# sumansamui/CMOOP_Audio_Processing

Measured on AMD Instinct MI355X. Metric: candidate-net evals/hour (pop=40, GSC-v2), higher is better.
Workload: dtype f32

## Files before the change

cmoop_audio_processing_amd/_lib.py:

```python
from __future__ import annotations

import ctypes as C
import os
import re
import subprocess
import threading

_HERE = os.path.dirname(os.path.abspath(__file__))
CSRC = os.path.join(_HERE, "csrc")
LIB_PATH = os.environ.get("CMOOP_LIB_PATH") or os.path.join(CSRC, "libcmoop_hip.so")
HEADER = os.path.join(os.path.dirname(_HERE), "include", "cmoop.h")

_lock = threading.Lock()
_lib = None


class CmoopError(RuntimeError):
    pass


class Config(C.Structure):
    _fields_ = [(n, C.c_int32) for n in (
        "variant", "classes", "epochs", "batch", "patience", "early_stop", "restore_best", "acc_readout",
        "fpr_variant", "shuffle", "eval_batch", "n_slots", "profile_every", "gemm_mode")] + \
        [(n, C.c_double) for n in ("lr", "beta1", "beta2", "adam_eps", "bn_eps", "bn_momentum", "dropout")]


class DatasetStruct(C.Structure):
    _fields_ = [("x_train", C.c_void_p), ("y_train", C.c_void_p), ("n_train", C.c_int64),
                ("x_val", C.c_void_p), ("y_val", C.c_void_p), ("n_val", C.c_int64),
                ("T", C.c_int32), ("F", C.c_int32)]


NEXT_FN = C.CFUNCTYPE(C.c_int32, C.c_void_p)


STREAM_PROTOTYPES = {
    "cmoop_net_predict": [C.c_void_p, C.c_void_p, C.c_int64, C.c_void_p],
    "cmoop_logmel_stream": [C.c_void_p, C.c_void_p, C.c_int64, C.c_void_p],
    "cmoop_logmel_stream_time": [C.c_void_p, C.c_void_p, C.c_int64, C.c_void_p, C.c_int32, C.c_void_p],
    "cmoop_stream_windows": [C.c_int64, C.c_int32, C.c_int32, C.c_void_p],
    "cmoop_net_predict_stream": [C.c_void_p, C.c_void_p, C.c_int64, C.c_int32, C.c_void_p, C.c_void_p, C.c_void_p, C.c_void_p],
}


def build(verbose: bool = False) -> str:
    jobs = str(min(8, os.cpu_count() or 1))
    r = subprocess.run(["make", "-C", CSRC, "-j", jobs], capture_output=True, text=True)
    if r.returncode != 0:
        raise CmoopError("building libcmoop_hip.so failed:\n" + r.stdout[-4000:] + r.stderr[-4000:])
    if verbose:
        print(r.stdout[-2000:])
    return LIB_PATH


def declared_symbols():
    txt = open(HEADER).read()
    return sorted(set(re.findall(r"\b(cmoop_[a-z0-9_]+)\s*\(", txt)))


def lib():
    global _lib
    with _lock:
        if _lib is not None:
            return _lib
        if not os.path.exists(LIB_PATH):
            raise CmoopError(
                f"{LIB_PATH} is missing: run `python -c 'import __graft_entry__ as g; g.build()'` "
                "(or `make -C cmoop_audio_processing_amd/csrc`). There is no CPU fallback for this path.")
        try:
            L = C.CDLL(LIB_PATH)
        except OSError as e:
            raise CmoopError(f"cannot load {LIB_PATH}: {e}") from e
        L.cmoop_last_error.restype = C.c_char_p
        L.cmoop_abi_version.restype = C.c_int
        for name in declared_symbols():
            fn = getattr(L, name)
            if name not in ("cmoop_last_error", "cmoop_config_default"):
                fn.restype = C.c_int
        L.cmoop_config_default.restype = None
        for name, argtypes in STREAM_PROTOTYPES.items():
            getattr(L, name).argtypes = argtypes
        _lib = L
        return L


def check(rc: int) -> None:
    if rc != 0:
        raise CmoopError(lib().cmoop_last_error().decode("utf-8", "replace"))


def default_config() -> Config:
    c = Config()
    lib().cmoop_config_default(C.byref(c))
    return c


def last_kernels():
    buf = C.create_string_buffer(1024)
    check(lib().cmoop_last_kernels(buf, C.c_int32(1024)))
    return [k for k in buf.value.decode().split(";") if k]


def profile_entries():
# ... 28 lines not shown
```

cmoop_audio_processing_amd/csrc/api.hip:

```cpp
#include "../../include/cmoop.h"
#include "net.h"

#include <cstring>
#include <memory>
#include <mutex>
#include <vector>

using namespace cmoop;

static thread_local std::string g_err;
static thread_local std::string g_last_kernels;

template <class F>
static int guard(F&& f) {
    try {
        f();
        return 0;
    } catch (const std::exception& e) {
        g_err = e.what();
        return 1;
    } catch (...) {
        g_err = "unknown error";
        return 2;
    }
// ... 739 lines not shown
                if (mfma_dgrad) {
                    CMOOP_HIP(hipMalloc(&wd, NK * 4));
                    launch_flip_transpose(w, wd, Cout, KS, KS, Cin, s);
                    if (KS * KS <= 32) {
                        tab_d_rows = rowtab_rows(gd);
                        CMOOP_HIP(hipMalloc(&tab_d, (size_t)tab_d_rows * 8));
                        launch_build_rowtab(gd, tab_d, s);
                    }
                    skf = igemm_splitk_workspace(gd);
                    if (skf) CMOOP_HIP(hipMalloc(&sk, skf * 4));
                }
                conv_backward_data(dy, w, dx, g, wd, mask_relu ? x : nullptr, 1.f, accumulate, s, &hook, sk, skf, GEMM_DEFAULT, mfma_dgrad,
                                   tab_d, tab_d_rows);
            }
            CMOOP_HIP(hipStreamSynchronize(s));
        } catch (...) {
            cleanup();
            throw;
        }
        cleanup();
    });
}

int cmoop_last_kernels(char* buf, int32_t cap) {
    return guard([&] {
        CMOOP_REQUIRE(buf && cap > 0, "last_kernels: no buffer");
        std::snprintf(buf, cap, "%s", g_last_kernels.c_str());
    });
}

int cmoop_conv_time(int32_t mode, const float* x, const float* w, const float* bias, float* y, int32_t B, int32_t H,
                    int32_t W, int32_t Cin, int32_t Cout, int32_t KS, int32_t iters, double* avg_ms) {
    return guard([&] {
        hipStream_t s = lib_stream();
        const ConvGeom g = make_geom(B, H, W, Cin, Cout, KS, 1);
        float *wd = nullptr, *wg = nullptr, *sk = nullptr;
        ConvGeom gd = g;
        GemmEpilogue e;
        const int S = wgrad_slices(g);
        if (mode == 0) e.bias = bias;
        if (mode == 1) {
            CMOOP_HIP(hipMalloc(&wd, (size_t)g.Cout * g.K() * 4));
            launch_flip_transpose(w, wd, Cout, KS, KS, Cin, s);
            gd.H = g.OH; gd.W = g.OW; gd.Cin = Cout; gd.Cout = Cin; gd.OH = g.H; gd.OW = g.W;
            gd.pad_t = KS - 1 - g.pad_t; gd.pad_l = KS - 1 - g.pad_l;
        }
// ... 68 lines not shown
```

cmoop_audio_processing_amd/csrc/gemm.hip:

```cpp
#include "kernels.h"
#include <hip/hip_ext.h>
#include <cstdlib>
#include <mutex>
#include <string>
#include <type_traits>

namespace cmoop {

typedef float f32x4 __attribute__((ext_vector_type(4)));

typedef __bf16 bf16x8 __attribute__((ext_vector_type(8)));
typedef unsigned u32x4 __attribute__((ext_vector_type(4)));

typedef __bf16 bf16x2 __attribute__((ext_vector_type(2)));
typedef float f32x2 __attribute__((ext_vector_type(2)));

template <int NP>
__device__ __forceinline__ void split_pair(const float x, const float y, unsigned (&w)[NP]) {
    if constexpr (NP == 1) {
        w[0] = __builtin_bit_cast(unsigned, __builtin_convertvector((f32x2){x, y}, bf16x2));
    } else {
        const unsigned ux = __float_as_uint(x), uy = __float_as_uint(y);
        w[0] = __builtin_amdgcn_perm(uy, ux, 0x07060302u);
        const float rx = x - __uint_as_float(ux & 0xFFFF0000u), ry = y - __uint_as_float(uy & 0xFFFF0000u);
// ... 1238 lines not shown
    if (c.halo) {
        c.mode = GEMM_FP32_HALO; c.use_dma = false;
        c.bm = halo_bm(cg.Cout);
        c.bn = std::min(cg.Cout, 64);
    } else if (halo_env && (c.mode == GEMM_FP32 || c.mode == GEMM_FP32_DMA) && c.bm == 128 && (c.splits > 1 || c.balanced_wgs) && ep.out_stride == 1) {
        int L = 0;
        const size_t need = halo_balanced_slab_floats(cg, &L);
        if (need > 0 && need <= ws_floats) {
            c.halo = true; c.halo_L = L; c.mode = GEMM_FP32_HALO; c.use_dma = false; c.stats = false;
            c.bm = 128; c.bn = 64; c.splits = 1; c.balanced_wgs = 512;
        }
    }
    c.flags = (c.splits > 1 ? GEMM_FLAG_SPLITK : 0) | (c.stats ? GEMM_FLAG_STATS : 0) | (c.balanced_wgs ? GEMM_FLAG_BALANCED : 0) |
              ((!c.halo && have_rowtab && (cg.Cin % bk) == 0 && cg.KH * cg.KW <= 32) ? GEMM_FLAG_ROWTAB : 0);
    return c;
}

int igemm_fwd_plan(const ConvGeom& g, const GemmEpilogue& ep, size_t ws_floats, bool want_stats, bool have_rowtab, int* flags_out) {
    igemm_check_range(g);
    CMOOP_REQUIRE(ilog2_exact(g.Cin) >= 4, "implicit GEMM needs C_in a power of two >= 16");
    const FwdChoice c = choose_fwd(g, ep, ws_floats, want_stats, have_rowtab);
    if (flags_out) *flags_out = c.flags;
    return c.code();
}

int launch_igemm_fwd(const float* X, const float* Wt, float* Y, const ConvGeom& cg, const GemmEpilogue& ep,
                     hipStream_t s, const GemmTiming* tm, float* splitk_ws, size_t splitk_ws_floats, int* stats_blocks,
                     const void* rowtab_v, int tab_rows, int* flags_out) {
    if (stats_blocks) *stats_blocks = 0;
    if (flags_out) *flags_out = 0;
    const uint2* rowtab = static_cast<const uint2*>(rowtab_v);
    GeomDev g = to_dev(cg);
    if (g.M == 0) return 0;
    EpiDev e;
    e.bias = ep.bias; e.mask = ep.mask; e.mask_scale = ep.mask_scale; e.relu = ep.relu;
    e.accumulate = ep.accumulate; e.out_stride = ep.out_stride; e.OHf = ep.OHf; e.OWf = ep.OWf;
    e.dropout = ep.dropout; e.drop_prefix = ep.drop_prefix; e.drop_thr = ep.drop_thr; e.drop_scale = ep.drop_scale;
    if (e.out_stride > 1)
        CMOOP_REQUIRE((int64_t)g.B * e.OHf * e.OWf * g.Cout < (1ll << 29), "scattered output too large");
    const FwdChoice ch = choose_fwd(cg, ep, splitk_ws ? splitk_ws_floats : 0, ep.stats != nullptr && stats_blocks != nullptr, rowtab != nullptr);
    const int mode = ch.mode == GEMM_FP32_DMA ? (int)GEMM_FP32 : ch.mode;
    const int bm = ch.bm, bn = ch.bn, splits = ch.splits, balanced_wgs = ch.balanced_wgs;
    const bool bk32_tile = ch.bk32_tile, use_dma = ch.use_dma;
    e.bal_L = 0; e.bal_segmax = 0;
    e.stats = ch.stats ? ep.stats : nullptr;
    if (e.stats) *stats_blocks = cdiv(g.M, bm);
// ... 902 lines not shown
```

cmoop_audio_processing_amd/csrc/kernels.h:

```cpp
#pragma once
#include "common.h"
#include <string>
#include <vector>

namespace cmoop {

struct ConvGeom {
    int B, H, W, Cin;
    int OH, OW, Cout;
    int KH, KW, stride;
    int pad_t, pad_l;
    int M() const { return B * OH * OW; }
    int K() const { return KH * KW * Cin; }
};

enum GemmMode { GEMM_DEFAULT = -1, GEMM_FP32 = 0, GEMM_FP32_DMA = 1 , GEMM_BF16X3 = 2, GEMM_BF16 = 3,
                GEMM_FP32_HALO = 4  };
int gemm_mode_default();

struct GemmEpilogue {
    int mode = GEMM_DEFAULT;
    const float* bias = nullptr;
    int relu = 0;
    const float* mask = nullptr;
    float mask_scale = 1.f;
    int accumulate = 0;
    int out_stride = 1;
    int OHf = 0, OWf = 0;
    int dropout = 0;
    uint32_t drop_prefix = 0, drop_thr = 0;
    float drop_scale = 1.f;
    float* stats = nullptr;
};

struct GemmTiming {
    hipEvent_t start = nullptr, stop = nullptr;
    bool ext = true;
};
enum GemmFlags { GEMM_FLAG_SPLITK = 1, GEMM_FLAG_STATS = 2, GEMM_FLAG_ROWTAB = 4, GEMM_FLAG_BALANCED = 8, GEMM_FLAG_SLABS = 16 };
int launch_igemm_fwd(const float* X, const float* Wt, float* Y, const ConvGeom& g,
                     const GemmEpilogue& e, hipStream_t s, const GemmTiming* tm = nullptr,
                     float* splitk_ws = nullptr, size_t splitk_ws_floats = 0, int* stats_blocks = nullptr,
                     const void* rowtab = nullptr, int tab_rows = 0, int* flags_out = nullptr);
size_t igemm_splitk_workspace(const ConvGeom& g);
int igemm_fwd_plan(const ConvGeom& g, const GemmEpilogue& e, size_t ws_floats, bool want_stats, bool have_rowtab, int* flags_out);
int igemm_wgrad_plan(const ConvGeom& g, int S, int mode, bool have_rowtab, int* flags_out);
void halo_rows_bound_and_need(const ConvGeom& g, int* bound, int* need, int* items_cap);
void igemm_check_range(const ConvGeom& g);
std::string gemm_kernel_name(int cls, int code);

int wgrad_slices(const ConvGeom& g);
int launch_igemm_wgrad(const float* X, const float* dY, float* P, const ConvGeom& g, int S, hipStream_t s,
                       const GemmTiming* tm = nullptr, float* Pbias = nullptr, size_t slab_stride = 0,
                       int mode = GEMM_DEFAULT, const void* rowtab = nullptr, int tab_rows = 0, int* flags_out = nullptr);
int rowtab_rows(const ConvGeom& g);
void launch_build_rowtab(const ConvGeom& g, void* tab, hipStream_t s);
void launch_reduce_slices(const float* P, float* out, int S, int64_t n, hipStream_t s, int64_t stride = 0);
void launch_flip_transpose(const float* W, float* Wd, int Cout, int KH, int KW, int Cin, hipStream_t s);
struct FlipEntry { int64_t w_off, wd_off; int Cout, KH, KW, Cin; };
void launch_flip_transpose_all(const float* params, float* wd_all, const FlipEntry* table_dev, int layers, int64_t max_elems,
                               hipStream_t s);

struct StepState {
    long long row0;
    unsigned step;
    unsigned iter;
};
void launch_step_advance(StepState* st, int batch, hipStream_t s);
void launch_glorot_init(float* w, int64_t n, uint32_t prefix, float scale, hipStream_t s);
void launch_fill(float* w, float v, int64_t n, hipStream_t s);

void launch_dense_fwd(const float* X, const float* W, const float* bias, float* Y, int M, int N, int K, int relu,
                      int dropout, uint32_t drop_prefix, uint32_t drop_thr, float drop_scale, int mode, hipStream_t s,
                      const StepState* st = nullptr, uint32_t drop_seed = 0, uint32_t drop_stream = 0);
void launch_dense_dgrad(const float* dY, const float* W, float* dX, int M, int N, int K, const float* mask, float mask_scale,
                        int mode, hipStream_t s);
void launch_dense_wgrad(const float* X, const float* dY, float* dW, float* dB, int M, int N, int K, int mode, hipStream_t s);
void launch_dense_bwd(const float* X, const float* dY, const float* W, float* dW, float* dB, float* dX, int M, int N, int K,
                      const float* mask, float mask_scale, int mode, hipStream_t s);

void launch_conv1_fwd(const float* X, const int32_t* idx, int64_t row0, const float* Wt, const float* bias,
                      float* Y, int B, int H, int W, int Cout, int KS, int relu, hipStream_t s, const StepState* st = nullptr,
                      int64_t n_rows = 0, float* stats = nullptr, int* stats_blocks = nullptr);
int conv1_wgrad_blocks(int B, int H, int W);
void launch_conv1_wgrad(const float* X, const int32_t* idx, int64_t row0, const float* dY, float* P,
                        int B, int H, int W, int Cout, int KS, hipStream_t s, const StepState* st = nullptr, int64_t n_rows = 0);

int colreduce_blocks(int64_t M, int C);
void launch_colstats(const float* X, float* P, int64_t M, int C, int blocks, hipStream_t s);
void launch_bn_bwd_reduce(const float* dY, const float* X, const float* mean, const float* invstd,
                          float* P, int64_t M, int C, int blocks, hipStream_t s);
void launch_bn_finalize(const float* P, int blocks, int64_t M, int C, const float* gamma, const float* beta,
                        float* moving_mean, float* moving_var, float* mean, float* invstd, float* scale,
// ... 82 lines not shown
```

cmoop_audio_processing_amd/csrc/net.h:

```cpp
#pragma once
#include "kernels.h"
#include <atomic>
#include <functional>
#include <map>
#include <mutex>
#include <set>
#include <string>
#include <vector>

namespace cmoop {

struct NetConfig {
    int variant = 0, classes = 10, epochs = 300, batch = 64, patience = 5;
    int early_stop = 1, restore_best = 0, acc_readout = 0, fpr_variant = 0, shuffle = 1;
    int eval_batch = 256, n_slots = 8, profile_every = 0;
    int gemm_mode = GEMM_FP32;
    double lr = 1e-3, beta1 = 0.9, beta2 = 0.999, adam_eps = 1e-7, bn_eps = 1e-3, bn_momentum = 0.99, dropout = 0.3;
};

struct Dataset {
    const float* x_train = nullptr; const int32_t* y_train = nullptr; int64_t n_train = 0;
    const float* x_val = nullptr;   const int32_t* y_val = nullptr;   int64_t n_val = 0;
    int T = 0, F = 0;
};
// ... 45 lines not shown
struct Op {
    OpKind kind;
    int in = -1, in2 = -1, out = -1;
    int KS = 1, stride = 1, Cin = 0, Cout = 0;
    int relu = 0, need_dgrad = 1, in_is_relu = 0, dgrad_accumulate = 0, dropout_layer = -1;
    float in_mask_scale = 1.f;
    int gemm_mode = GEMM_FP32;
    void* rowtab = nullptr;
    int rowtab_rows = 0;
    void* rowtab_d = nullptr;
    int rowtab_d_rows = 0;
    int64_t w_off = 0, b_off = 0, wd_off = -1;
    int64_t slab_off = -1;
    size_t slab_floats = 0;
    int tensor_index = 0;
    int64_t gamma_off = 0, beta_off = 0, mm_off = 0, mv_off = 0;
    int relu_after = 0, mask_in_pos = 0;
    int fuse_pool = 0;
    int feeds_bn = 0;
    float* bn_buf = nullptr;
    uint8_t* arg = nullptr;
    int mask_y_pos = 0;
    int fused_into_bn = 0;
};

class Net : public GemmHook {
  public:
    const GemmTiming* begin(int cls, double flops) override;
    void end(int code, int flags) override;
    Net(const int32_t gene[6], const NetConfig& cfg, int T, int F, uint32_t seed, hipStream_t stream);
    ~Net();
    Net(const Net&) = delete;
    Net& operator=(const Net&) = delete;

    int64_t total_params() const { return n_params_; }
    void get_params(float* host);
    void set_params(const float* host);
    void get_grads(float* host);
    void snapshot_params();
    void restore_snapshot();
    void get_state(float* params, float* m, float* v, long long* iterations, long long* steps);
    void set_state(const float* params, const float* m, const float* v, long long iterations, long long steps);
    void set_gather_rows(int64_t n) { gather_rows_ = n; }
    void run_epoch(const float* X, const int32_t* y, int64_t n_train, int epoch, int32_t* idx_scratch);

    void train_step(const float* X, const int32_t* y, const int32_t* idx, int64_t row0, int B);
    void begin_fit(int64_t total_steps);
    void begin_epoch();
    void train_step_stateful(const float* X, const int32_t* y, const int32_t* idx, int B);
    void evaluate(const float* X, const int32_t* y, int64_t n, double* loss_sum, long long* correct, int32_t* preds);
    void predict(const float* X, int64_t n, float* probs);
    void predict_stream(const float* feat, int64_t n_frames, int hop, bool db_scale, bool db_ref_max, float db_amin, float top_db,
                        const double* mean, const double* scale, float* probs);
    void read_train_metrics(double* loss_sum, long long* correct, bool reset);
    void drain_profile();
    hipStream_t stream() const { return stream_; }
    uint32_t seed() const { return seed_; }
    const NetConfig& config() const { return cfg_; }
    int feature_T() const { return T_; }
    int feature_F() const { return F_; }
    long long steps_done() const { return step_; }
    long long iterations_done() const { return iterations_; }

  private:
    void build_plan();
    void forward(const float* X, const int32_t* idx, int64_t row0, int B, bool train, const StepState* st = nullptr);
    void backward(const float* X, const int32_t* idx, int64_t row0, int B, const StepState* st = nullptr);
    void step_body(const float* X, const int32_t* y, const int32_t* idx, int64_t row0, int B, const StepState* st);
    ConvGeom geom_of(const Op& op, int B) const;
    void run_gemm(int cls, const float* X, const float* Wt, float* Y, const ConvGeom& g, const GemmEpilogue& e, int* stats_blocks = nullptr,
                  const void* rowtab = nullptr, int tab_rows = 0);
    float* dalloc(size_t floats);

    int32_t gene_[6];
    NetConfig cfg_;
    int T_, F_, Bmax_;
    uint32_t seed_;
    hipStream_t stream_;
    std::vector<Act> acts_;
    std::vector<Op> ops_;
    std::vector<void*> allocs_;
    int64_t n_params_ = 0;
    float *params_ = nullptr, *grads_ = nullptr, *adam_m_ = nullptr, *adam_v_ = nullptr, *snap_ = nullptr;
    float *wgrad_ws_ = nullptr, *wd_ws_ = nullptr, *red_ws_ = nullptr, *splitk_ws_ = nullptr;
    StepState* st_dev_ = nullptr;
    float* alpha_tab_ = nullptr;
    int64_t alpha_tab_n_ = 0, host_row0_ = 0, gather_rows_ = 0;
    hipGraphExec_t graph_exec_ = nullptr;
    bool graph_ok_ = true;
    FlipEntry* flip_table_ = nullptr;
    int flip_layers_ = 0;
    int64_t flip_max_elems_ = 0;
    std::vector<AdamSeg> slab_segs_;
    size_t wgrad_ws_floats_ = 0, wd_ws_floats_ = 0, red_ws_floats_ = 0, splitk_ws_floats_ = 0;
    double* acc_train_ = nullptr;
    double* acc_eval_ = nullptr;
    int logits_ = -1;
    long long step_ = 0, iterations_ = 0;
    bool profiling_now_ = false, hook_live_ = false;
    int fused_stats_blocks_ = 0;
    struct EvPair { GemmTiming t; double flops; int cls, code, flags; };
    std::vector<EvPair> ev_pool_;
    size_t ev_used_ = 0;
};

struct EvalResult {
    double acc = 0, size_mb = 0, fpr = 0, val_loss = 0, seconds = 0;
    int epochs_run = 0;
    int evaluated = 0;
};

struct FitHistory {
// ... 15 lines not shown
```

cmoop_audio_processing_amd/csrc/net.hip:

```cpp
#include "net.h"

#include <algorithm>
#include <chrono>
#include <cmath>
#include <cstdlib>
#include <cstring>
#include <functional>
#include <map>
#include <numeric>
#include <thread>

namespace cmoop {

static const int FC_LADDER[5][4] = {{0, 0, 0, 0}, {64, 0, 0, 0}, {128, 64, 0, 0}, {256, 128, 64, 0}, {512, 256, 128, 64}};

void validate_gene(const int32_t g[6]) {
    const bool ok = (g[0] == 16 || g[0] == 32 || g[0] == 64) && (g[1] == 3 || g[1] == 5) && (g[2] == 0 || g[2] == 1) &&
                    (g[3] >= 1 && g[3] <= 3) && (g[4] >= 1 && g[4] <= 4) && (g[5] == 0 || g[5] == 1);
    CMOOP_REQUIRE(ok, "gene outside the search space (filters{16,32,64}, kernel{3,5}, bn{0,1}, res{1..3}, fc{1..4}, dropout{0,1})");
}

int64_t param_count(const int32_t g[6], int variant, int classes) {
    validate_gene(g);
    const int64_t f = g[0], kk = (int64_t)g[1] * g[1], bn = g[2], R = g[3], fc = g[4];
// ... 205 lines not shown
        if (fuse_ok && !ops_.empty() && ops_.back().kind == OP_BN && ops_.back().out == in && !mask_y_pos) {
            ops_.back().fuse_pool = 1;
            op.fused_into_bn = 1;
            acts_[in].virt = true;
        }
        const Act ia = acts_[in];
        op.out = new_act((ia.H + 1) / 2, (ia.W + 1) / 2, ia.C);
        ops_.push_back(op);
        return op.out;
    };

    int x;
    if (A) {
        x = add_conv(OP_CONV1, 0, f, k, 1, !bn, 0, 1.f, 0);
        if (bn) x = add_bn(x, 1, 0);
        x = add_conv(OP_CONV, x, f, k, 1, !bn, 1, 1.f, 0);
        if (bn) x = add_bn(x, 1, 0);
        x = add_pool(x, 0);
    } else {
        x = add_conv(OP_CONV1, 0, f, k, 1, 1, 0, 1.f, 0);
        if (bn) x = add_bn(x, 0, 1);
        x = add_pool(x, !bn);
    }
    int c = f;
    for (int r = 0; r < R; ++r) {
        const int in_relu = (A || r > 0) ? 1 : 0;
        const int skip = add_conv(OP_CONV, x, 2 * c, 1, 2, 0, in_relu, 1.f, 1);
        int y;
        if (A) {
            y = add_conv(OP_CONV, x, 2 * c, k, 1, !bn, in_relu, 1.f, 0);
            if (bn) y = add_bn(y, 1, 0);
            y = add_conv(OP_CONV, y, 2 * c, k, 1, 0, 1, 1.f, 0);
            if (bn) y = add_bn(y, 0, 0);
            y = add_pool(y, 0);
        } else {
            y = add_conv(OP_CONV, x, 2 * c, k, 1, 1, in_relu, 1.f, 0);
            if (bn) y = add_bn(y, 0, 1);
            y = add_pool(y, !bn);
        }
        Op op; op.kind = OP_ADDRELU; op.in = y; op.in2 = skip;
        op.out = new_act(acts_[y].H, acts_[y].W, acts_[y].C);
        ops_.push_back(op);
        x = op.out;
        c *= 2;
    }
    {
        Op op; op.kind = OP_GAP; op.in = x;
        op.out = new_act(1, 1, acts_[x].C);
        ops_.push_back(op);
        x = op.out;
    }
    const float keep_scale = (float)(1.0 / (1.0 - cfg_.dropout));
    for (int i = 0; i < fc; ++i) {
        const int in_relu = i > 0;
        const float ms = (in_relu && dr) ? keep_scale : 1.f;
        x = add_conv(OP_DENSE, x, FC_LADDER[fc][i], 1, 1, 1, in_relu, ms, 0);
        if (dr) ops_.back().dropout_layer = i;
    }
    x = add_conv(OP_DENSE, x, cfg_.classes, 1, 1, 0, 1, dr ? keep_scale : 1.f, 0);
    ops_.back().gemm_mode = GEMM_FP32;
    logits_ = x;
    n_params_ = off;
    CMOOP_REQUIRE(n_params_ == param_count(gene_, cfg_.variant, cfg_.classes), "plan / closed-form parameter count mismatch");
// ... 106 lines not shown
        ev_pool_.resize(1024);
        const char* pm = std::getenv("CMOOP_PROFILE_PAIRS");
        const bool ext = !(pm && pm[0] == '1');
        static std::atomic<bool> said{false};
        if (!said.exchange(true)) std::fprintf(stderr, "[cmoop] GEMM launch timing: %s\n", ext ? "hipExtLaunchKernelGGL events" : "hipEventRecord pairs");
        for (auto& e : ev_pool_) {
            CMOOP_HIP(hipEventCreate(&e.t.start));
            CMOOP_HIP(hipEventCreate(&e.t.stop));
            e.t.ext = ext;
        }
    }
}

ConvGeom Net::geom_of(const Op& op, int B) const {
    const Act& ia = acts_[op.in];
    ConvGeom g;
    g.B = B; g.H = ia.H; g.W = ia.W; g.Cin = op.Cin;
    g.OH = (ia.H + op.stride - 1) / op.stride; g.OW = (ia.W + op.stride - 1) / op.stride; g.Cout = op.Cout;
    g.KH = g.KW = op.KS; g.stride = op.stride;
    const int th = std::max((g.OH - 1) * op.stride + op.KS - ia.H, 0);
    const int tw = std::max((g.OW - 1) * op.stride + op.KS - ia.W, 0);
    g.pad_t = th / 2; g.pad_l = tw / 2;
    return g;
}

void Net::get_params(float* host) {
    CMOOP_HIP(hipMemcpyAsync(host, params_, n_params_ * 4, hipMemcpyDeviceToHost, stream_));
    CMOOP_HIP(hipStreamSynchronize(stream_));
}
void Net::set_params(const float* host) {
    CMOOP_HIP(hipMemcpyAsync(params_, host, n_params_ * 4, hipMemcpyHostToDevice, stream_));
    CMOOP_HIP(hipStreamSynchronize(stream_));
}
void Net::get_grads(float* host) {
    CMOOP_HIP(hipMemcpyAsync(host, grads_, n_params_ * 4, hipMemcpyDeviceToHost, stream_));
    CMOOP_HIP(hipStreamSynchronize(stream_));
}
void Net::snapshot_params() {
    if (!snap_) snap_ = dalloc(n_params_);
    CMOOP_HIP(hipMemcpyAsync(snap_, params_, n_params_ * 4, hipMemcpyDeviceToDevice, stream_));
}
void Net::restore_snapshot() {
    if (snap_) CMOOP_HIP(hipMemcpyAsync(params_, snap_, n_params_ * 4, hipMemcpyDeviceToDevice, stream_));
}

const GemmTiming* Net::begin(int cls, double flops) {
// ... 111 lines not shown
            const std::string name = gemm_kernel_name(ev_pool_[i].cls, ev_pool_[i].code);
            t.variants.insert(gemm_variant_name(ev_pool_[i].cls, ev_pool_[i].code, ev_pool_[i].flags));
            ProfileEntry& e = t.by_kernel[name];
            e.ms += ms;
            e.flops += ev_pool_[i].flops;
            e.launches += 1;
        }
    }
    ev_used_ = 0;
}

void Net::forward(const float* X, const int32_t* idx, int64_t row0, int B, bool train, const StepState* st) {
    CMOOP_REQUIRE(B >= 1 && B <= Bmax_, "batch larger than the net was planned for");
    for (size_t oi = 0; oi < ops_.size(); ++oi) {
        const Op& op = ops_[oi];
        switch (op.kind) {
        case OP_CONV1:
            fused_stats_blocks_ = 0;
            launch_conv1_fwd(X, idx, row0, params_ + op.w_off, params_ + op.b_off, acts_[op.out].data, B, T_, F_, op.Cout,
                             op.KS, op.relu, stream_, st, train ? gather_rows_ : 0, (train && op.feeds_bn) ? red_ws_ : nullptr,
                             (train && op.feeds_bn) ? &fused_stats_blocks_ : nullptr);
            break;
        case OP_CONV: {
            GemmEpilogue e;
            e.mode = op.gemm_mode;
            e.bias = params_ + op.b_off;
            e.relu = op.relu;
            fused_stats_blocks_ = 0;
            if (train && op.feeds_bn) e.stats = red_ws_;
            run_gemm(0, acts_[op.in].data, params_ + op.w_off, acts_[op.out].data, geom_of(op, B), e,
                     e.stats ? &fused_stats_blocks_ : nullptr, op.rowtab, op.rowtab_rows);
            break;
        }
        case OP_DENSE: {
            const bool drop = train && op.dropout_layer >= 0;
            launch_dense_fwd(acts_[op.in].data, params_ + op.w_off, params_ + op.b_off, acts_[op.out].data, B, op.Cout, op.Cin,
                             op.relu, drop ? 1 : 0,
                             drop ? rng_prefix(seed_, STREAM_DROPOUT + (uint32_t)op.dropout_layer, (uint32_t)step_) : 0u,
                             (uint32_t)(cfg_.dropout * 16777216.0), (float)(1.0 / (1.0 - cfg_.dropout)), op.gemm_mode, stream_,
                             drop ? st : nullptr, seed_, drop ? STREAM_DROPOUT + (uint32_t)op.dropout_layer : 0u);
            break;
        }
        case OP_BN: {
            const Act& ia = acts_[op.in];
            const int64_t M = (int64_t)B * ia.H * ia.W;
            const int C = op.Cout;
// ... 6 lines not shown
                    launch_colstats(ia.data, red_ws_, M, C, nb, stream_);
                }
                launch_bn_finalize(red_ws_, nb, M, C, params_ + op.gamma_off, params_ + op.beta_off, params_ + op.mm_off,
                                   params_ + op.mv_off, mean, invstd, scale, shift, (float)cfg_.bn_eps, (float)cfg_.bn_momentum,
                                   (float)(1.0 - cfg_.bn_momentum), stream_);
            } else {
                launch_bn_eval_prepare(params_ + op.gamma_off, params_ + op.beta_off, params_ + op.mm_off,
                                       params_ + op.mv_off, scale, shift, C, (float)cfg_.bn_eps, stream_);
            }
            if (op.fuse_pool) {
                const Op& pool = ops_[oi + 1];
                launch_bn_pool_fwd(ia.data, acts_[pool.out].data, pool.arg, scale, shift, B, ia.H, ia.W, C, op.relu_after, stream_);
            } else {
                launch_scale_shift(ia.data, acts_[op.out].data, scale, shift, M, C, op.relu_after, stream_);
            }
            break;
        }
        case OP_POOL: {
            if (op.fused_into_bn) break;
            const Act& ia = acts_[op.in];
            launch_maxpool_fwd(ia.data, acts_[op.out].data, op.arg, B, ia.H, ia.W, ia.C, stream_);
            break;
        }
        case OP_ADDRELU:
            launch_add_relu(acts_[op.in].data, acts_[op.in2].data, acts_[op.out].data,
                            (int64_t)B * acts_[op.out].per_sample(), stream_);
            break;
        case OP_GAP: {
            const Act& ia = acts_[op.in];
            launch_gap_fwd(ia.data, acts_[op.out].data, B, ia.H * ia.W, ia.C, stream_);
            break;
        }
        }
    }
}

void Net::backward(const float* X, const int32_t* idx, int64_t row0, int B, const StepState* st) {
    slab_segs_.clear();
    launch_flip_transpose_all(params_, wd_ws_, flip_table_, flip_layers_, flip_max_elems_, stream_);
    for (int oi = (int)ops_.size() - 1; oi >= 0; --oi) {
        const Op& op = ops_[oi];
        switch (op.kind) {
        case OP_DENSE: {
            const float* dY = acts_[op.out].grad;
            Act& ia = acts_[op.in];
            const char* du = std::getenv("CMOOP_DENSE_UNFUSED");
            const bool unfused = du && du[0] == '1';
            if (op.need_dgrad && !unfused) {
                launch_dense_bwd(ia.data, dY, params_ + op.w_off, grads_ + op.w_off, grads_ + op.b_off, ia.grad, B, op.Cout, op.Cin,
                                 op.in_is_relu ? ia.data : nullptr, op.in_mask_scale, op.gemm_mode, stream_);
                break;
            }
            launch_dense_wgrad(ia.data, dY, grads_ + op.w_off, grads_ + op.b_off, B, op.Cout, op.Cin, op.gemm_mode, stream_);
            if (op.need_dgrad)
                launch_dense_dgrad(dY, params_ + op.w_off, ia.grad, B, op.Cout, op.Cin, op.in_is_relu ? ia.data : nullptr,
                                   op.in_mask_scale, op.gemm_mode, stream_);
            break;
        }
        case OP_CONV: {
            const ConvGeom g = geom_of(op, B);
            const float* dY = acts_[op.out].grad;
            Act& ia = acts_[op.in];
            AdamSeg sg;
            sg.off = op.w_off;
            conv_backward_weights(ia.data, dY, grads_ + op.w_off, grads_ + op.b_off, g, wgrad_ws_ + op.slab_off, op.slab_floats, stream_,
                                  this, op.gemm_mode, op.rowtab, op.rowtab_rows, &sg);
            if (sg.slab) slab_segs_.push_back(sg);
            if (op.need_dgrad)
                conv_backward_data(dY, params_ + op.w_off, ia.grad, g, wd_ws_ + op.wd_off, op.in_is_relu ? ia.data : nullptr,
                                   op.in_mask_scale, op.dgrad_accumulate, stream_, this, splitk_ws_, splitk_ws_floats_, op.gemm_mode,
                                   true, op.rowtab_d, op.rowtab_d_rows);
            break;
        }
        case OP_BN: {
            const Act& ia = acts_[op.in];
            const int64_t M = (int64_t)B * ia.H * ia.W;
            const int C = op.Cout;
            float *mean = op.bn_buf, *invstd = mean + C;
            const int nb = colreduce_blocks(M, C);
            if (op.fuse_pool) {
                const Op& pool = ops_[oi + 1];
                launch_bn_pool_bwd_reduce(acts_[pool.out].grad, pool.arg, ia.data, mean, invstd, red_ws_, B, ia.H, ia.W, C, nb, stream_);
                launch_bn_pool_bwd_apply(acts_[pool.out].grad, pool.arg, ia.data, mean, invstd, params_ + op.gamma_off, red_ws_, nb,
                                         ia.grad, grads_ + op.gamma_off, grads_ + op.beta_off, B, ia.H, ia.W, C, op.mask_in_pos, stream_);
                break;
            }
            launch_bn_bwd_reduce(acts_[op.out].grad, ia.data, mean, invstd, red_ws_, M, C, nb, stream_);
            launch_bn_bwd_apply(acts_[op.out].grad, ia.data, mean, invstd, params_ + op.gamma_off, red_ws_, nb, ia.grad,
                                grads_ + op.gamma_off, grads_ + op.beta_off, M, C, op.mask_in_pos, stream_);
            break;
        }
// ... 456 lines not shown
```

include/cmoop.h:

```cpp
#ifndef CMOOP_H
#define CMOOP_H

#include <stdint.h>

#ifdef __cplusplus
extern "C" {
#endif

#define CMOOP_ABI_VERSION 3

#define CMOOP_VARIANT_A 0
#define CMOOP_VARIANT_B 1

#define CMOOP_FPR_V1 0
#define CMOOP_FPR_V1_QUIRK 1
#define CMOOP_FPR_V3 2

#define CMOOP_GEMM_DEFAULT 0
#define CMOOP_GEMM_BF16X3 2
#define CMOOP_GEMM_BF16 3

typedef struct cmoop_config {
    int32_t variant;
    int32_t classes;
// ... 102 lines not shown
int cmoop_net_predict_stream(cmoop_net* net, const float* feat_dev, int64_t n_frames, int32_t hop_frames,
                             const cmoop_frontend_config* db, const double* mean_host, const double* scale_host,
                             float* probs_dev);
int cmoop_net_get_state(cmoop_net* net, float* params, float* adam_m, float* adam_v, int64_t* iterations, int64_t* steps);
int cmoop_net_set_state(cmoop_net* net, const float* params, const float* adam_m, const float* adam_v, int64_t iterations,
                        int64_t steps);
int cmoop_net_set_gather_rows(cmoop_net* net, int64_t n_rows);
int cmoop_net_run_epoch(cmoop_net* net, const float* x_train_dev, const int32_t* y_train_dev, int64_t n_train, int32_t epoch);
int cmoop_net_fit(cmoop_net* net, const cmoop_dataset* ds, int32_t hist_cap, double* val_loss_hist, double* val_acc_hist,
                  int32_t* epochs_run, int32_t* best_epoch, double* acc, double* fpr, double* val_loss);
int cmoop_epoch_permutation(uint32_t seed, uint32_t epoch, int64_t n, int32_t* out_host);
int cmoop_epoch_permutation_device(uint32_t seed, uint32_t epoch, int64_t n, int32_t* out_dev);

int cmoop_conv_fwd(const float* x_dev, const float* w_dev, const float* bias_dev, float* y_dev, int32_t B, int32_t H,
                   int32_t W, int32_t Cin, int32_t Cout, int32_t KS, int32_t stride, int32_t relu);
int cmoop_conv_bwd(const float* x_dev, const float* w_dev, const float* dy_dev, float* dx_dev, float* dw_dev, float* db_dev,
                   int32_t B, int32_t H, int32_t W, int32_t Cin, int32_t Cout, int32_t KS, int32_t stride, int32_t mask_relu);
int cmoop_conv_fwd_trainer(const float* x_dev, const float* w_dev, const float* bias_dev, float* y_dev, int32_t B, int32_t H,
                           int32_t W, int32_t Cin, int32_t Cout, int32_t KS, int32_t stride, int32_t relu, double* col_sum,
                           double* col_sumsq, int32_t* stats_fused);
int cmoop_conv_bwd_trainer(const float* x_dev, const float* w_dev, const float* dy_dev, float* dx_dev, float* dw_dev,
                           float* db_dev, int32_t B, int32_t H, int32_t W, int32_t Cin, int32_t Cout, int32_t KS, int32_t stride,
                           int32_t mask_relu);
int cmoop_last_kernels(char* buf, int32_t cap);
int cmoop_conv_time(int32_t mode, const float* x_dev, const float* w_dev, const float* bias_dev, float* y_dev, int32_t B,
                    int32_t H, int32_t W, int32_t Cin, int32_t Cout, int32_t KS, int32_t iters, double* avg_ms);
int cmoop_dense_fwd(const float* x_dev, const float* w_dev, const float* bias_dev, float* y_dev, int32_t M, int32_t N, int32_t K,
                    int32_t relu);
int cmoop_dense_bwd(const float* x_dev, const float* w_dev, const float* dy_dev, float* dx_dev, float* dw_dev, float* db_dev,
                    int32_t M, int32_t N, int32_t K, int32_t mask_relu);
int cmoop_maxpool_fwd(const float* x_dev, float* y_dev, uint8_t* arg_dev, int32_t B, int32_t H, int32_t W, int32_t C);
int cmoop_maxpool_bwd(const float* dy_dev, const uint8_t* arg_dev, const float* y_dev, float* dx_dev, int32_t B, int32_t H,
                      int32_t W, int32_t C, int32_t mask_y_pos);
int cmoop_device_synchronize(void);

#ifdef __cplusplus
}
#endif
#endif
```

Measured before the change: 440.9.

## Fuse residual 1x1 stride-2 skip conv with add-ReLU and dgrad accumulate

Adds a dedicated MFMA kernel for the 1x1 stride-2 residual projection. In the forward pass it computes the skip conv, bias, residual add and ReLU in one launch, deferring the conv to the ADDRELU op. In backward it does the strided dgrad with the ReLU mask and accumulation into the input gradient directly. This removes the separate skip activation write and read, the add_relu pass and the general implicit-GEMM launch. It mirrors the split-K chain of the general GEMM so the rounding order matches. The risk is that the simpler kernel may run slower than the tuned igemm for some shapes, and it adds new entry points.

```diff
diff --git a/cmoop_audio_processing_amd/_lib.py b/cmoop_audio_processing_amd/_lib.py
--- a/cmoop_audio_processing_amd/_lib.py
+++ b/cmoop_audio_processing_amd/_lib.py
@@ -44,6 +44,14 @@
 }
 
 
+SKIP_PROTOTYPES = {
+    "cmoop_skip_plan": [C.c_int32] * 6 + [C.c_void_p, C.c_void_p],
+    "cmoop_skip_fwd": [C.c_void_p] * 5 + [C.c_int32] * 5,
+    "cmoop_skip_dgrad": [C.c_void_p] * 4 + [C.c_int32] * 6,
+    "cmoop_skip_time": [C.c_int32] + [C.c_void_p] * 7 + [C.c_int32] * 6 + [C.c_void_p],
+}
+
+
 def build(verbose: bool = False) -> str:
     jobs = str(min(8, os.cpu_count() or 1))
     r = subprocess.run(["make", "-C", CSRC, "-j", jobs], capture_output=True, text=True)
@@ -79,7 +87,7 @@
             if name not in ("cmoop_last_error", "cmoop_config_default"):
                 fn.restype = C.c_int
         L.cmoop_config_default.restype = None
-        for name, argtypes in STREAM_PROTOTYPES.items():
+        for name, argtypes in list(STREAM_PROTOTYPES.items()) + list(SKIP_PROTOTYPES.items()):
             getattr(L, name).argtypes = argtypes
         _lib = L
         return L
diff --git a/cmoop_audio_processing_amd/csrc/api.hip b/cmoop_audio_processing_amd/csrc/api.hip
--- a/cmoop_audio_processing_amd/csrc/api.hip
+++ b/cmoop_audio_processing_amd/csrc/api.hip
@@ -785,6 +785,115 @@
     });
 }
 
+static size_t skip_twin_workspace(const ConvGeom& g, int op) { return igemm_splitk_workspace(op == 0 ? g : dgrad_geometry(g)); }
+
+int cmoop_skip_plan(int32_t op, int32_t B, int32_t H, int32_t W, int32_t Cin, int32_t Cout, int32_t* fused, int32_t* splits) {
+    return guard([&] {
+        CMOOP_REQUIRE(fused && splits && (op == 0 || op == 1), "skip_plan: bad arguments");
+        CMOOP_REQUIRE(B >= 1 && H >= 1 && W >= 1 && Cin >= 1 && Cout >= 1, "bad conv shape");
+        const ConvGeom g = make_geom(B, H, W, Cin, Cout, 1, 2);
+        SkipChain c;
+        const bool ok = op == 0 ? skip_fwd_chain(g, GEMM_DEFAULT, skip_twin_workspace(g, 0), &c)
+                                : skip_dgrad_chain(g, GEMM_DEFAULT, skip_twin_workspace(g, 1), &c);
+        *fused = ok ? 1 : 0;
+        *splits = ok ? c.splits : 0;
+    });
+}
+
+int cmoop_skip_fwd(const float* x, const float* w, const float* bias, const float* p, float* y, int32_t B, int32_t H, int32_t W,
+                   int32_t Cin, int32_t Cout) {
+    return guard([&] {
+        CMOOP_REQUIRE(B >= 1 && H >= 1 && W >= 1 && Cin >= 1 && Cout >= 1, "bad conv shape");
+        hipStream_t s = lib_stream();
+        const ConvGeom g = make_geom(B, H, W, Cin, Cout, 1, 2);
+        SkipChain c;
+        CMOOP_REQUIRE(skip_fwd_chain(g, GEMM_DEFAULT, skip_twin_workspace(g, 0), &c), "skip_fwd: the fused kernel does not serve this launch");
+        launch_skip_fwd(x, w, bias, p, y, g, c, s);
+        CMOOP_HIP(hipStreamSynchronize(s));
+    });
+}
+
+int cmoop_skip_dgrad(const float* x, const float* w, const float* dy, float* dx, int32_t B, int32_t H, int32_t W, int32_t Cin,
+                     int32_t Cout, int32_t mask_relu) {
+    return guard([&] {
+        CMOOP_REQUIRE(B >= 1 && H >= 1 && W >= 1 && Cin >= 1 && Cout >= 1, "bad conv shape");
+        CMOOP_REQUIRE(!mask_relu || x, "skip_dgrad: the ReLU mask needs x");
+        hipStream_t s = lib_stream();
+        const ConvGeom g = make_geom(B, H, W, Cin, Cout, 1, 2);
+        SkipChain c;
+        CMOOP_REQUIRE(skip_dgrad_chain(g, GEMM_DEFAULT, skip_twin_workspace(g, 1), &c), "skip_dgrad: the fused kernel does not serve this launch");
+        float* wd = nullptr;
+        CMOOP_HIP(hipMalloc(&wd, (size_t)Cout * Cin * 4));
+        try {
+            launch_flip_transpose(w, wd, Cout, 1, 1, Cin, s);
+            launch_skip_dgrad(dy, wd, dx, g, mask_relu ? x : nullptr, 1.f, c, s);
+            CMOOP_HIP(hipStreamSynchronize(s));
+        } catch (...) {
+            hipStreamSynchronize(s);
+            hipFree(wd);
+            throw;
+        }
+        hipFree(wd);
+    });
+}
+
+int cmoop_skip_time(int32_t mode, const float* x, const float* w, const float* bias, const float* p, float* y, const float* dy,
+                    float* dx, int32_t B, int32_t H, int32_t W, int32_t Cin, int32_t Cout, int32_t iters, double* avg_ms) {
+    return guard([&] {
+        CMOOP_REQUIRE(avg_ms && mode >= 0 && mode <= 3 && B >= 1 && H >= 1 && W >= 1 && Cin >= 16 && Cout >= 16, "skip_time: bad arguments");
+        hipStream_t s = lib_stream();
+        const ConvGeom g = make_geom(B, H, W, Cin, Cout, 1, 2);
+        const ConvGeom gd = dgrad_geometry(g);
+        const bool bwd = mode == 1 || mode == 3;
+        SkipChain c;
+        if (mode == 0) CMOOP_REQUIRE(skip_fwd_chain(g, GEMM_DEFAULT, skip_twin_workspace(g, 0), &c), "skip_time: not served by the fused forward");
+        if (mode == 1) CMOOP_REQUIRE(skip_dgrad_chain(g, GEMM_DEFAULT, skip_twin_workspace(g, 1), &c), "skip_time: not served by the fused dgrad");
+        float *wd = nullptr, *sk = nullptr;
+        void* tab = nullptr;
+        hipEvent_t a = nullptr, b = nullptr;
+        auto cleanup = [&] { hipStreamSynchronize(s); if (wd) hipFree(wd); if (sk) hipFree(sk); if (tab) hipFree(tab); if (a) hipEventDestroy(a); if (b) hipEventDestroy(b); };
+        try {
+            if (bwd) {
+                CMOOP_HIP(hipMalloc(&wd, (size_t)Cout * Cin * 4));
+                launch_flip_transpose(w, wd, Cout, 1, 1, Cin, s);
+            }
+            const int tab_rows = mode >= 2 ? rowtab_rows(bwd ? gd : g) : 0;
+            if (tab_rows) {
+                CMOOP_HIP(hipMalloc(&tab, (size_t)tab_rows * 8));
+                launch_build_rowtab(bwd ? gd : g, tab, s);
+            }
+            const size_t skf = mode >= 2 ? skip_twin_workspace(g, bwd ? 1 : 0) : 0;
+            if (skf) CMOOP_HIP(hipMalloc(&sk, skf * 4));
+            auto once = [&]() {
+                if (mode == 0) launch_skip_fwd(x, w, bias, p, y, g, c, s);
+                else if (mode == 1) launch_skip_dgrad(dy, wd, dx, g, x, 1.f, c, s);
+                else if (mode == 2) {
+                    GemmEpilogue e;
+                    e.bias = bias;
+                    launch_igemm_fwd(x, w, y, g, e, s, nullptr, sk, skf, nullptr, tab, tab_rows);
+                    launch_add_relu(p, y, y, (int64_t)g.M() * Cout, s);
+                } else {
+                    conv_backward_data(dy, w, dx, g, wd, x, 1.f, 1, s, nullptr, sk, skf, GEMM_DEFAULT, true, tab, tab_rows);
+                }
+            };
+            for (int i = 0; i < 3; ++i) once();
+            CMOOP_HIP(hipEventCreate(&a));
+            CMOOP_HIP(hipEventCreate(&b));
+            CMOOP_HIP(hipEventRecord(a, s));
+            for (int i = 0; i < iters; ++i) once();
+            CMOOP_HIP(hipEventRecord(b, s));
+            CMOOP_HIP(hipEventSynchronize(b));
+            float ms = 0.f;
+            CMOOP_HIP(hipEventElapsedTime(&ms, a, b));
+            *avg_ms = (double)ms / std::max(1, iters);
+        } catch (...) {
+            cleanup();
+            throw;
+        }
+        cleanup();
+    });
+}
+
 int cmoop_last_kernels(char* buf, int32_t cap) {
     return guard([&] {
         CMOOP_REQUIRE(buf && cap > 0, "last_kernels: no buffer");
diff --git a/cmoop_audio_processing_amd/csrc/gemm.hip b/cmoop_audio_processing_amd/csrc/gemm.hip
--- a/cmoop_audio_processing_amd/csrc/gemm.hip
+++ b/cmoop_audio_processing_amd/csrc/gemm.hip
@@ -1284,6 +1284,17 @@
     const FwdChoice c = choose_fwd(g, ep, ws_floats, want_stats, have_rowtab);
     if (flags_out) *flags_out = c.flags;
     return c.code();
+}
+
+bool igemm_fwd_chain(const ConvGeom& g, const GemmEpilogue& ep, size_t ws_floats, bool have_rowtab, int* splits, int* chunks_per_split,
+                     int* bk) {
+    if (ilog2_exact(g.Cin) < 4) return false;
+    const FwdChoice c = choose_fwd(g, ep, ws_floats, false, have_rowtab);
+    if ((c.mode != GEMM_FP32 && c.mode != GEMM_FP32_DMA) || c.balanced_wgs || c.halo) return false;
+    *bk = c.bk32_tile ? 32 : 16;
+    *splits = c.splits;
+    *chunks_per_split = cdiv(cdiv(g.K(), *bk), c.splits);
+    return true;
 }
 
 int launch_igemm_fwd(const float* X, const float* Wt, float* Y, const ConvGeom& cg, const GemmEpilogue& ep,
diff --git a/cmoop_audio_processing_amd/csrc/kernels.h b/cmoop_audio_processing_amd/csrc/kernels.h
--- a/cmoop_audio_processing_amd/csrc/kernels.h
+++ b/cmoop_audio_processing_amd/csrc/kernels.h
@@ -45,6 +45,8 @@
 size_t igemm_splitk_workspace(const ConvGeom& g);
 int igemm_fwd_plan(const ConvGeom& g, const GemmEpilogue& e, size_t ws_floats, bool want_stats, bool have_rowtab, int* flags_out);
 int igemm_wgrad_plan(const ConvGeom& g, int S, int mode, bool have_rowtab, int* flags_out);
+bool igemm_fwd_chain(const ConvGeom& g, const GemmEpilogue& e, size_t ws_floats, bool have_rowtab, int* splits, int* chunks_per_split,
+                     int* bk);
 void halo_rows_bound_and_need(const ConvGeom& g, int* bound, int* need, int* items_cap);
 void igemm_check_range(const ConvGeom& g);
 std::string gemm_kernel_name(int cls, int code);
@@ -69,6 +71,14 @@
 void launch_step_advance(StepState* st, int batch, hipStream_t s);
 void launch_glorot_init(float* w, int64_t n, uint32_t prefix, float scale, hipStream_t s);
 void launch_fill(float* w, float v, int64_t n, hipStream_t s);
+
+struct SkipChain { int splits = 1, piece_groups = 0; };
+bool skip_fwd_chain(const ConvGeom& g, int mode, size_t ws_floats, SkipChain* c);
+bool skip_dgrad_chain(const ConvGeom& g, int mode, size_t ws_floats, SkipChain* c);
+void launch_skip_fwd(const float* X, const float* Wt, const float* bias, const float* P, float* Y, const ConvGeom& g,
+                     const SkipChain& c, hipStream_t s);
+void launch_skip_dgrad(const float* dY, const float* Wd, float* dX, const ConvGeom& g, const float* mask, float mask_scale,
+                       const SkipChain& c, hipStream_t s);
 
 void launch_dense_fwd(const float* X, const float* W, const float* bias, float* Y, int M, int N, int K, int relu,
                       int dropout, uint32_t drop_prefix, uint32_t drop_thr, float drop_scale, int mode, hipStream_t s,
diff --git a/cmoop_audio_processing_amd/csrc/net.h b/cmoop_audio_processing_amd/csrc/net.h
--- a/cmoop_audio_processing_amd/csrc/net.h
+++ b/cmoop_audio_processing_amd/csrc/net.h
@@ -91,6 +91,8 @@
     uint8_t* arg = nullptr;
     int mask_y_pos = 0;
     int fused_into_bn = 0;
+    int is_skip = 0;
+    int skip_op = -1;
 };
 
 class Net : public GemmHook {
@@ -137,6 +139,8 @@
     void backward(const float* X, const int32_t* idx, int64_t row0, int B, const StepState* st = nullptr);
     void step_body(const float* X, const int32_t* y, const int32_t* idx, int64_t row0, int B, const StepState* st);
     ConvGeom geom_of(const Op& op, int B) const;
+    bool skip_fwd_fused(const Op& op, int B, SkipChain* c) const;
+    bool skip_dgrad_fused(const Op& op, int B, SkipChain* c) const;
     void run_gemm(int cls, const float* X, const float* Wt, float* Y, const ConvGeom& g, const GemmEpilogue& e, int* stats_blocks = nullptr,
                   const void* rowtab = nullptr, int tab_rows = 0);
     float* dalloc(size_t floats);
@@ -157,6 +161,7 @@
     int64_t alpha_tab_n_ = 0, host_row0_ = 0, gather_rows_ = 0;
     hipGraphExec_t graph_exec_ = nullptr;
     bool graph_ok_ = true;
+    bool skip_fused_ = true;
     FlipEntry* flip_table_ = nullptr;
     int flip_layers_ = 0;
     int64_t flip_max_elems_ = 0;
diff --git a/cmoop_audio_processing_amd/csrc/net.hip b/cmoop_audio_processing_amd/csrc/net.hip
--- a/cmoop_audio_processing_amd/csrc/net.hip
+++ b/cmoop_audio_processing_amd/csrc/net.hip
@@ -251,10 +251,16 @@
         if (bn) x = add_bn(x, 0, 1);
         x = add_pool(x, !bn);
     }
+    {
+        const char* sf = std::getenv("CMOOP_SKIP_FUSED");
+        skip_fused_ = !(sf && sf[0] == '0');
+    }
     int c = f;
     for (int r = 0; r < R; ++r) {
         const int in_relu = (A || r > 0) ? 1 : 0;
         const int skip = add_conv(OP_CONV, x, 2 * c, 1, 2, 0, in_relu, 1.f, 1);
+        const int skip_op = (int)ops_.size() - 1;
+        ops_[skip_op].is_skip = 1;
         int y;
         if (A) {
             y = add_conv(OP_CONV, x, 2 * c, k, 1, !bn, in_relu, 1.f, 0);
@@ -268,6 +274,7 @@
             y = add_pool(y, !bn);
         }
         Op op; op.kind = OP_ADDRELU; op.in = y; op.in2 = skip;
+        op.skip_op = skip_op;
         op.out = new_act(acts_[y].H, acts_[y].W, acts_[y].C);
         ops_.push_back(op);
         x = op.out;
@@ -420,6 +427,13 @@
     const int tw = std::max((g.OW - 1) * op.stride + op.KS - ia.W, 0);
     g.pad_t = th / 2; g.pad_l = tw / 2;
     return g;
+}
+
+bool Net::skip_fwd_fused(const Op& op, int B, SkipChain* c) const {
+    return skip_fused_ && op.is_skip && skip_fwd_chain(geom_of(op, B), op.gemm_mode, splitk_ws_ ? splitk_ws_floats_ : 0, c);
+}
+bool Net::skip_dgrad_fused(const Op& op, int B, SkipChain* c) const {
+    return skip_fused_ && op.is_skip && skip_dgrad_chain(geom_of(op, B), op.gemm_mode, splitk_ws_ ? splitk_ws_floats_ : 0, c);
 }
 
 void Net::get_params(float* host) {
@@ -577,6 +591,8 @@
                              (train && op.feeds_bn) ? &fused_stats_blocks_ : nullptr);
             break;
         case OP_CONV: {
+            SkipChain sc;
+            if (skip_fwd_fused(op, B, &sc)) break;
             GemmEpilogue e;
             e.mode = op.gemm_mode;
             e.bias = params_ + op.b_off;
@@ -629,10 +645,18 @@
             launch_maxpool_fwd(ia.data, acts_[op.out].data, op.arg, B, ia.H, ia.W, ia.C, stream_);
             break;
         }
-        case OP_ADDRELU:
+        case OP_ADDRELU: {
+            const Op& sk = ops_[op.skip_op];
+            SkipChain sc;
+            if (skip_fwd_fused(sk, B, &sc)) {
+                launch_skip_fwd(acts_[sk.in].data, params_ + sk.w_off, params_ + sk.b_off, acts_[op.in].data, acts_[op.out].data,
+                                geom_of(sk, B), sc, stream_);
+                break;
+            }
             launch_add_relu(acts_[op.in].data, acts_[op.in2].data, acts_[op.out].data,
                             (int64_t)B * acts_[op.out].per_sample(), stream_);
             break;
+        }
         case OP_GAP: {
             const Act& ia = acts_[op.in];
             launch_gap_fwd(ia.data, acts_[op.out].data, B, ia.H * ia.W, ia.C, stream_);
@@ -673,7 +697,10 @@
             conv_backward_weights(ia.data, dY, grads_ + op.w_off, grads_ + op.b_off, g, wgrad_ws_ + op.slab_off, op.slab_floats, stream_,
                                   this, op.gemm_mode, op.rowtab, op.rowtab_rows, &sg);
             if (sg.slab) slab_segs_.push_back(sg);
-            if (op.need_dgrad)
+            SkipChain sc;
+            if (op.need_dgrad && op.dgrad_accumulate && skip_dgrad_fused(op, B, &sc))
+                launch_skip_dgrad(dY, wd_ws_ + op.wd_off, ia.grad, g, op.in_is_relu ? ia.data : nullptr, op.in_mask_scale, sc, stream_);
+            else if (op.need_dgrad)
                 conv_backward_data(dY, params_ + op.w_off, ia.grad, g, wd_ws_ + op.wd_off, op.in_is_relu ? ia.data : nullptr,
                                    op.in_mask_scale, op.dgrad_accumulate, stream_, this, splitk_ws_, splitk_ws_floats_, op.gemm_mode,
                                    true, op.rowtab_d, op.rowtab_d_rows);
diff --git a/cmoop_audio_processing_amd/csrc/skip.hip b/cmoop_audio_processing_amd/csrc/skip.hip
--- /dev/null
+++ b/cmoop_audio_processing_amd/csrc/skip.hip
@@ -0,0 +1,238 @@
+#include "net.h"
+
+namespace cmoop {
+
+typedef float f32x4 __attribute__((ext_vector_type(4)));
+
+struct SkipDev {
+    int M, N, K;
+    int OHW, OW, H, W;
+    int nct;
+    int piece_groups;
+};
+
+template <int G, int RT, bool DGRAD>
+__global__ __launch_bounds__(256) void skip_kernel(const float* __restrict__ A, const float* __restrict__ Wt,
+                                                   const float* __restrict__ bias, const float* __restrict__ P, float* Y,
+                                                   SkipDev d, float mask_scale) {
+    constexpr int CT = 2;
+    const int wave = threadIdx.x >> 6, lane = threadIdx.x & 63, lr = lane & 15, q = lane >> 4;
+    const int tile = blockIdx.x * 4 + wave;
+    const int mt = tile / d.nct, nt = tile - mt * d.nct;
+    const int m0 = mt * (16 * RT), n0 = nt * 32;
+    if (m0 >= d.M) return;
+
+    auto pixel = [&](int row) {
+        const int b = row / d.OHW, rr = row - b * d.OHW;
+        const int oh = rr / d.OW, ow = rr - oh * d.OW;
+        return (size_t)(b * d.H + 2 * oh) * d.W + 2 * ow;
+    };
+
+    const float* ap[RT];
+    const float* bp[CT];
+#pragma unroll
+    for (int rt = 0; rt < RT; ++rt) {
+        const int row = min(m0 + rt * 16 + lr, d.M - 1);
+        ap[rt] = A + (DGRAD ? (size_t)row : pixel(row)) * d.K + 4 * q;
+    }
+#pragma unroll
+    for (int ct = 0; ct < CT; ++ct) bp[ct] = Wt + (size_t)min(n0 + ct * 16 + lr, d.N - 1) * d.K + 4 * q;
+
+    const bool masked = DGRAD && P != nullptr;
+    const float* Pc = DGRAD ? (masked ? P : Y) : P;
+    size_t off[RT][4];
+    int colc[CT];
+    bool rok[RT][4], cok[CT];
+    float pv[RT][4][CT], old[RT][4][CT], bias_v[CT];
+#pragma unroll
+    for (int ct = 0; ct < CT; ++ct) {
+        const int col = n0 + ct * 16 + lr;
+        cok[ct] = col < d.N;
+        colc[ct] = min(col, d.N - 1);
+        bias_v[ct] = DGRAD ? 0.f : bias[colc[ct]];
+    }
+#pragma unroll
+    for (int rt = 0; rt < RT; ++rt)
+#pragma unroll
+        for (int r = 0; r < 4; ++r) {
+            const int row = m0 + rt * 16 + q * 4 + r;
+            rok[rt][r] = row < d.M;
+            const int rc = min(row, d.M - 1);
+            off[rt][r] = (DGRAD ? pixel(rc) : (size_t)rc) * d.N;
+#pragma unroll
+            for (int ct = 0; ct < CT; ++ct) {
+                pv[rt][r][ct] = Pc[off[rt][r] + colc[ct]];
+                old[rt][r][ct] = DGRAD ? Y[off[rt][r] + colc[ct]] : 0.f;
+            }
+        }
+
+    f32x4 acc[RT][CT], tot[RT][CT];
+#pragma unroll
+    for (int i = 0; i < RT; ++i)
+#pragma unroll
+        for (int j = 0; j < CT; ++j) {
+            acc[i][j] = f32x4{0.f, 0.f, 0.f, 0.f};
+            tot[i][j] = f32x4{0.f, 0.f, 0.f, 0.f};
+        }
+    const bool split = d.piece_groups > 0;
+    int left = split ? d.piece_groups : 0x7fffffff;
+    auto close_piece = [&]() {
+#pragma unroll
+        for (int i = 0; i < RT; ++i)
+#pragma unroll
+            for (int j = 0; j < CT; ++j) {
+                tot[i][j] += acc[i][j];
+                acc[i][j] = f32x4{0.f, 0.f, 0.f, 0.f};
+            }
+        left = d.piece_groups;
+    };
+
+    auto load = [&](int c, f32x4 (&a)[RT][G], f32x4 (&b)[CT][G]) {
+#pragma unroll
+        for (int gi = 0; gi < G; ++gi) {
+#pragma unroll
+            for (int rt = 0; rt < RT; ++rt) a[rt][gi] = *reinterpret_cast<const f32x4*>(ap[rt] + (c * G + gi) * 16);
+#pragma unroll
+            for (int ct = 0; ct < CT; ++ct) b[ct][gi] = *reinterpret_cast<const f32x4*>(bp[ct] + (c * G + gi) * 16);
+        }
+    };
+    auto compute = [&](const f32x4 (&a)[RT][G], const f32x4 (&b)[CT][G]) {
+#pragma unroll
+        for (int gi = 0; gi < G; ++gi) {
+#pragma unroll
+            for (int j = 0; j < 4; ++j)
+#pragma unroll
+                for (int rt = 0; rt < RT; ++rt)
+#pragma unroll
+                    for (int ct = 0; ct < CT; ++ct)
+                        acc[rt][ct] = __builtin_amdgcn_mfma_f32_16x16x4f32(a[rt][gi][j], b[ct][gi][j], acc[rt][ct], 0, 0, 0);
+            if (--left == 0) close_piece();
+        }
+    };
+
+    f32x4 a0[RT][G], b0[CT][G];
+    load(0, a0, b0);
+    if constexpr (G < 8) {
+        compute(a0, b0);
+    } else {
+        f32x4 a1[RT][G], b1[CT][G];
+        const int nch = d.K / (16 * G);
+        for (int c = 0; c < nch; c += 2) {
+            if (c + 1 < nch) load(c + 1, a1, b1);
+            compute(a0, b0);
+            if (c + 1 >= nch) break;
+            if (c + 2 < nch) load(c + 2, a0, b0);
+            compute(a1, b1);
+        }
+    }
+    if (split && left != d.piece_groups) close_piece();
+
+    float res[RT][4][CT];
+#pragma unroll
+    for (int rt = 0; rt < RT; ++rt)
+#pragma unroll
+        for (int r = 0; r < 4; ++r)
+#pragma unroll
+            for (int ct = 0; ct < CT; ++ct) {
+                float v = (split ? tot[rt][ct][r] : acc[rt][ct][r]) + bias_v[ct];
+                if constexpr (DGRAD) {
+                    if (masked) v = (pv[rt][r][ct] > 0.f) ? v * mask_scale : 0.f;
+                    v += old[rt][r][ct];
+                } else {
+                    v = fmaxf(pv[rt][r][ct] + v, 0.f);
+                }
+                res[rt][r][ct] = v;
+            }
+    if (m0 + 16 * RT <= d.M && n0 + 32 <= d.N) {
+#pragma unroll
+        for (int rt = 0; rt < RT; ++rt)
+#pragma unroll
+            for (int r = 0; r < 4; ++r)
+#pragma unroll
+                for (int ct = 0; ct < CT; ++ct) Y[off[rt][r] + colc[ct]] = res[rt][r][ct];
+    } else {
+#pragma unroll
+        for (int rt = 0; rt < RT; ++rt)
+#pragma unroll
+            for (int r = 0; r < 4; ++r)
+#pragma unroll
+                for (int ct = 0; ct < CT; ++ct)
+                    if (rok[rt][r] && cok[ct]) Y[off[rt][r] + colc[ct]] = res[rt][r][ct];
+    }
+}
+
+template <bool DGRAD>
+static void launch_skip_t(const float* A, const float* Wt, const float* bias, const float* P, float* Y, const SkipDev& d,
+                          float mask_scale, hipStream_t s) {
+    if (d.M == 0) return;
+    const int groups = d.K / 16;
+    const bool rt2 = (long)cdiv(d.M, 32) * d.nct >= 1024;
+    const long tiles = (long)cdiv(d.M, rt2 ? 32 : 16) * d.nct;
+    const dim3 grid((unsigned)((tiles + 3) / 4)), block(256);
+#define CMOOP_SKIP(G_)                                                                                             \
+    do {                                                                                                           \
+        if (rt2) hipLaunchKernelGGL((skip_kernel<G_, 2, DGRAD>), grid, block, 0, s, A, Wt, bias, P, Y, d, mask_scale); \
+        else hipLaunchKernelGGL((skip_kernel<G_, 1, DGRAD>), grid, block, 0, s, A, Wt, bias, P, Y, d, mask_scale);     \
+    } while (0)
+    if (groups >= 8) CMOOP_SKIP(8);
+    else if (groups == 4) CMOOP_SKIP(4);
+    else if (groups == 2) CMOOP_SKIP(2);
+    else CMOOP_SKIP(1);
+#undef CMOOP_SKIP
+    CMOOP_HIP(hipGetLastError());
+}
+
+static bool skip_shape_ok(const ConvGeom& g) {
+    return g.KH == 1 && g.KW == 1 && g.stride == 2 && g.pad_t == 0 && g.pad_l == 0 && g.OH == (g.H + 1) / 2 && g.OW == (g.W + 1) / 2 &&
+           ilog2_exact(g.Cin) >= 4 && ilog2_exact(g.Cout) >= 4 && g.Cin <= 512 && g.Cout <= 512;
+}
+
+static bool chain_of(const ConvGeom& gemm, const GemmEpilogue& e, size_t ws_floats, SkipChain* c) {
+    int splits = 1, cps = 0, bk = 0;
+    if (!igemm_fwd_chain(gemm, e, ws_floats, true, &splits, &cps, &bk)) return false;
+    c->splits = splits;
+    c->piece_groups = splits > 1 ? cps * (bk / 16) : 0;
+    return true;
+}
+
+bool skip_fwd_chain(const ConvGeom& g, int mode, size_t ws_floats, SkipChain* c) {
+    if (!skip_shape_ok(g)) return false;
+    GemmEpilogue e;
+    e.mode = mode;
+    return chain_of(g, e, ws_floats, c);
+}
+
+bool skip_dgrad_chain(const ConvGeom& g, int mode, size_t ws_floats, SkipChain* c) {
+    if (!skip_shape_ok(g)) return false;
+    GemmEpilogue e;
+    e.mode = mode;
+    e.out_stride = g.stride; e.OHf = g.H; e.OWf = g.W;
+    e.accumulate = 1;
+    return chain_of(dgrad_geometry(g), e, ws_floats, c);
+}
+
+static SkipDev skip_dev(const ConvGeom& g, bool dgrad, const SkipChain& c) {
+    CMOOP_REQUIRE(skip_shape_ok(g), "skip kernels: not a 1x1 stride-2 projection with power-of-two channels in [16, 512]");
+    igemm_check_range(g);
+    SkipDev d;
+    d.M = g.M(); d.N = dgrad ? g.Cin : g.Cout; d.K = dgrad ? g.Cout : g.Cin;
+    d.OHW = g.OH * g.OW; d.OW = g.OW; d.H = g.H; d.W = g.W;
+    d.nct = cdiv(d.N, 32);
+    d.piece_groups = c.splits > 1 ? c.piece_groups : 0;
+    CMOOP_REQUIRE(d.piece_groups >= 0 && d.piece_groups <= d.K / 16, "skip kernels: bad split-K chain");
+    return d;
+}
+
+void launch_skip_fwd(const float* X, const float* Wt, const float* bias, const float* P, float* Y, const ConvGeom& g,
+                     const SkipChain& c, hipStream_t s) {
+    CMOOP_REQUIRE(X && Wt && bias && P && Y, "skip forward: NULL operand");
+    launch_skip_t<false>(X, Wt, bias, P, Y, skip_dev(g, false, c), 1.f, s);
+}
+
+void launch_skip_dgrad(const float* dY, const float* Wd, float* dX, const ConvGeom& g, const float* mask, float mask_scale,
+                       const SkipChain& c, hipStream_t s) {
+    CMOOP_REQUIRE(dY && Wd && dX, "skip dgrad: NULL operand");
+    launch_skip_t<true>(dY, Wd, nullptr, mask, dX, skip_dev(g, true, c), mask_scale, s);
+}
+
+}
diff --git a/include/cmoop.h b/include/cmoop.h
--- a/include/cmoop.h
+++ b/include/cmoop.h
@@ -148,6 +148,14 @@
 int cmoop_conv_bwd_trainer(const float* x_dev, const float* w_dev, const float* dy_dev, float* dx_dev, float* dw_dev,
                            float* db_dev, int32_t B, int32_t H, int32_t W, int32_t Cin, int32_t Cout, int32_t KS, int32_t stride,
                            int32_t mask_relu);
+int cmoop_skip_plan(int32_t op, int32_t B, int32_t H, int32_t W, int32_t Cin, int32_t Cout, int32_t* fused, int32_t* splits);
+int cmoop_skip_fwd(const float* x_dev, const float* w_dev, const float* bias_dev, const float* p_dev, float* y_dev, int32_t B,
+                   int32_t H, int32_t W, int32_t Cin, int32_t Cout);
+int cmoop_skip_dgrad(const float* x_dev, const float* w_dev, const float* dy_dev, float* dx_dev, int32_t B, int32_t H, int32_t W,
+                     int32_t Cin, int32_t Cout, int32_t mask_relu);
+int cmoop_skip_time(int32_t mode, const float* x_dev, const float* w_dev, const float* bias_dev, const float* p_dev, float* y_dev,
+                    const float* dy_dev, float* dx_dev, int32_t B, int32_t H, int32_t W, int32_t Cin, int32_t Cout, int32_t iters,
+                    double* avg_ms);
 int cmoop_last_kernels(char* buf, int32_t cap);
 int cmoop_conv_time(int32_t mode, const float* x_dev, const float* w_dev, const float* bias_dev, float* y_dev, int32_t B,
                     int32_t H, int32_t W, int32_t Cin, int32_t Cout, int32_t KS, int32_t iters, double* avg_ms);
```

Result: no change. 443.8, median of 6 (+0.7%).
